# LongTarget/Fasim-LongTarget

Measured on AMD Instinct MI355X. Metric: SW Gcells/s (logical, whole job: stage 1+2+3 of the triplex scan), higher is better.
Workload: dtype u8

## Files before the change

### fasim-longtarget_amd/csrc/align.hip

```cpp
#include <hip/hip_runtime.h>
#include <stdint.h>
#include <stdlib.h>
#include "kernels.h"

namespace fasim {

typedef short v2s __attribute__((ext_vector_type(2)));
typedef unsigned short v2u __attribute__((ext_vector_type(2)));
typedef int v4i __attribute__((ext_vector_type(4)));

__device__ __forceinline__ v2s a_s(v2u x) { return __builtin_bit_cast(v2s, x); }
__device__ __forceinline__ v2u a_u(v2s x) { return __builtin_bit_cast(v2u, x); }
__device__ __forceinline__ int a_i(v2s x) { return __builtin_bit_cast(int, x); }
__device__ __forceinline__ int a_i(v2u x) { return __builtin_bit_cast(int, x); }
__device__ __forceinline__ v2u u_from(int x) { return __builtin_bit_cast(v2u, x); }
__device__ __forceinline__ v2s s_fromi(int x) { return __builtin_bit_cast(v2s, x); }

__device__ __forceinline__ v2u apk_subs(v2u a, v2u b) { v2u r; asm("v_pk_sub_u16 %0, %1, %2 clamp" : "=v"(r) : "v"(a), "v"(b)); return r; }
__device__ __forceinline__ v2u apk_subs_k(v2u a, uint32_t k) { v2u r; asm("v_pk_sub_u16 %0, %1, %2 clamp" : "=v"(r) : "v"(a), "s"(k)); return r; }
__device__ __forceinline__ v2u apk_ksubs(uint32_t k, v2u a) { v2u r; asm("v_pk_sub_u16 %0, %1, %2 clamp" : "=v"(r) : "s"(k), "v"(a)); return r; }
__device__ __forceinline__ v2u apk_minu(v2u a, v2u b) { v2u r; asm("v_pk_min_u16 %0, %1, %2" : "=v"(r) : "v"(a), "v"(b)); return r; }
__device__ __forceinline__ v2u apk_minu_k(v2u a, uint32_t k) { v2u r; asm("v_pk_min_u16 %0, %1, %2" : "=v"(r) : "v"(a), "s"(k)); return r; }
__device__ __forceinline__ v2u apk_maxu(v2u a, v2u b) { v2u r; asm("v_pk_max_u16 %0, %1, %2" : "=v"(r) : "v"(a), "v"(b)); return r; }

// ... 706 lines not shown
		if (i + band < end) end = i + band;
		if (j < beg || j > end) { status = 3; break; }
		const uint32_t nib = dir[(int64_t)(width_d * i + (j - x)) * 64];
		int dv;
		const int dE = (nib & 1) ? 3 : 2, dF = (nib & 2) ? 5 : 4;
		if (state == 0) dv = dE; else if (state == 1) dv = dF; else { const int dh = (nib >> 2) & 3; dv = dh == 0 ? 1 : (dh == 1 ? dE : dF); }
		if (dv == 1) { --i; --j; state = 2; op = 0; }
		else if (dv == 2) { --i; state = 0; op = 1; }
		else if (dv == 3) { --i; state = 2; op = 1; }
		else if (dv == 4) { --j; state = 1; op = 2; }
		else { --j; state = 2; op = 2; }
		if (op == prev_op) ++e;
		else {
			if (l >= ALIGN_MAX_CIGAR) { status = 4; break; }
			rc[l++] = cig(e, prev_op);
			prev_op = op; e = 1;
		}
	}
	if (status == 0) {
		if (op == 0) { if (l >= ALIGN_MAX_CIGAR) status = 4; else rc[l++] = cig(e + 1, 0); }
		else { if (l + 2 > ALIGN_MAX_CIGAR) status = 4; else { rc[l++] = cig(e, op); rc[l++] = cig(1, 0); } }
	}
	if (status == 0) {
		const uint32_t off = atomicAdd(pool_count, (uint32_t)l);
		if ((uint64_t)off + (uint64_t)l > (uint64_t)pool_cap) status = 4;
		else { o->cigar_off = off; for (int k = 0; k < l; k++) cigar_pool[off + k] = rc[l - 1 - k]; }
	}
	o->status = status;
	if (status != 0) return;
	o->sw_score = score;
	o->cigar_len = l;
}

hipError_t launch_finish(const uint8_t* tcodes, const uint8_t* qcodes, const FwdProb* probs, const FwdOut* fwd, const int32_t* order,
	int32_t nprob, uint8_t* dirs, AlignOutDev* out, uint32_t* cigar_pool, uint32_t pool_cap, uint32_t* pool_count, hipStream_t st)
{
	if (nprob <= 0) return hipSuccess;
	hipError_t err = hipMemsetAsync(pool_count, 0, sizeof(uint32_t), st);
	if (err != hipSuccess) return err;
	hipLaunchKernelGGL((k_finish_lds<64, 2048>), dim3((nprob + 63) / 64), dim3(64), 0, st, tcodes, qcodes, probs, fwd, order, nprob, dirs, out,
		cigar_pool, pool_cap, pool_count);
	return hipGetLastError();
}

hipError_t launch_finish_mid(const uint8_t* tcodes, const uint8_t* qcodes, const FwdProb* probs, const FwdOut* fwd, const int32_t* idx_list,
	int32_t nlist, uint8_t* dirs, AlignOutDev* out, uint32_t* cigar_pool, uint32_t pool_cap, uint32_t* pool_count, hipStream_t st)
{
	if (nlist <= 0) return hipSuccess;
	static bool attr_set = false;
	if (!attr_set) { (void)hipFuncSetAttribute((const void*)k_finish_lds<256, 16384>, hipFuncAttributeMaxDynamicSharedMemorySize, 64 * 1024); attr_set = true; }
	hipLaunchKernelGGL((k_finish_lds<256, 16384>), dim3((nlist + 63) / 64), dim3(64), 0, st, tcodes, qcodes, probs, fwd, idx_list, nlist, dirs, out,
		cigar_pool, pool_cap, pool_count);
	return hipGetLastError();
}

hipError_t launch_finish_big(const uint8_t* tcodes, const uint8_t* qcodes, const FwdProb* probs, const FwdOut* fwd,
	const int32_t* idx_list, int32_t nlist, uint8_t* scratch, int32_t scratch_cap, AlignOutDev* out, uint32_t* cigar_pool,
	uint32_t pool_cap, uint32_t* pool_count, hipStream_t st)
{
	if (nlist <= 0) return hipSuccess;
	hipLaunchKernelGGL(k_finish, dim3((nlist + 63) / 64), dim3(64), 0, st, tcodes, qcodes, probs, fwd, nlist, scratch, scratch_cap, out,
		cigar_pool, pool_cap, pool_count, idx_list);
	return hipGetLastError();
}

}
```

### fasim-longtarget_amd/csrc/engine.cpp

```cpp
#include "engine.h"

extern "C" {

void fasim_params_default(fasim_params* p)
{
	p->rule = 0; p->cutLength = 5000; p->strand = 0; p->overlapLength = 100; p->ntMin = 20; p->ntMax = 100000;
	p->scoreMin = 0.0f; p->minIdentity = 60.0f; p->minStability = 1.0f; p->penaltyT = -1000; p->penaltyC = 0;
	p->cDistance = 15; p->cLength = 50; p->classicSim = 0;
}

const char* fasim_last_error(const fasim_engine* e) { return e ? e->err.c_str() : g_last_error.c_str(); }

int fasim_engine_create(int device, fasim_engine** out) { return fasim_engine_create_ex(device, 0, out); }

int fasim_engine_create_ex(int device, int32_t flags, fasim_engine** out)
{
	if (!out) return fail(nullptr, FASIM_E_ARG, "null out pointer");
	*out = nullptr;
	const bool tune = !(flags & FASIM_CREATE_NO_PROCESS_TUNING);
	if (tune) setenv("GPU_MAX_HW_QUEUES", "8", 0);
	if (tune) {
		static const bool once = [] {
			const char* e = getenv("FASIM_MALLOPT");
			if (e && atoi(e) == 0) return false;
			(void)mallopt(M_MMAP_THRESHOLD, 32 * 1024 * 1024);
			(void)mallopt(M_TRIM_THRESHOLD, 0x7fffffff);
			(void)mallopt(M_TOP_PAD, 256 * 1024 * 1024);
			return true;
		}();
		(void)once;
	}
	int count = 0;
	hipError_t he = hipGetDeviceCount(&count);
	if (he != hipSuccess || count <= 0) return fail(nullptr, FASIM_E_NODEVICE, "no HIP device available (%s); this library has no CPU fallback", hipGetErrorString(he));
	if (device < 0 || device >= count) return fail(nullptr, FASIM_E_NODEVICE, "device %d out of range (%d devices)", device, count);
	{
		const char* e = getenv("FASIM_BLOCKING_SYNC");
		if (tune && !(e && atoi(e) == 0)) { (void)hipSetDevice(device); (void)hipSetDeviceFlags(hipDeviceScheduleBlockingSync); (void)hipGetLastError(); }
	}
	fasim_engine* E = new fasim_engine();
	E->device = device;
	he = hipSetDevice(device);
	if (he == hipSuccess) he = hipStreamCreate(&E->st);
	if (he != hipSuccess) { int rc = fail(nullptr, FASIM_E_NODEVICE, "cannot initialise device %d: %s", device, hipGetErrorString(he)); delete E; return rc; }
	E->lut1 = make_lut(true); E->lut2 = make_lut(false);
	std::vector<uint8_t> lut(48 * 256);
	build_enc_lut(lut.data());
	if (upload(E, E->enc_lut, lut.data(), lut.size()) || E->counter.ensure(64) != hipSuccess) { delete E; return FASIM_E_HIP; }
	unsigned hc = std::thread::hardware_concurrency();
	const char* env = getenv("FASIM_HOST_THREADS");
	E->host_threads = env ? std::max(1, atoi(env)) : (int)std::min(96u, std::max(1u, hc * 3 / 8));
	E->host_threads_total = E->host_threads;
	E->host_threads_explicit = env != nullptr;
	const char* v1 = getenv("FASIM_SCAN_V1");
	E->scan_v1 = v1 && atoi(v1) != 0;
	const char* a1 = getenv("FASIM_ALIGN_V1");
	E->align_v1 = a1 && atoi(a1) != 0;
	const char* sw = getenv("FASIM_STRIPED_WINDOW");
	E->striped_window = sw && atoi(sw) != 0;
	*out = E;
	return FASIM_OK;
}

void fasim_engine_destroy(fasim_engine* e)
{
	if (!e) return;
	for (fasim_engine* w : e->workers) fasim_engine_destroy(w);
	e->workers.clear();
	(void)hipSetDevice(e->device);
	DevBuf* bufs[] = { &e->q1, &e->q2, &e->enc_lut, &e->counter, &e->dna, &e->seg_start, &e->seg_len, &e->enc_ids, &e->tcodes,
		&e->colmax, &e->probs, &e->max_out, &e->unit_len, &e->stage1, &e->hits, &e->hits_total, &e->hit_off, &e->hit_cnt, &e->thr,
		&e->ends, &e->bprobs, &e->bout, &e->scratch, &e->dna_res, &e->colmax16, &e->unit_ids, &e->flags, &e->stage1_in, &e->hits2,
		&e->fprobs, &e->ftasks, &e->fstream, &e->fout, &e->aout, &e->cigpool, &e->cigcount, &e->forder, &e->scratch2, &e->boundary, &e->fboundary, &e->unit_hz,
		&e->unit_first, &e->hz_cols, &e->hz_plan, &e->hz_base, &e->hz_items, &e->snap, &e->hz_state, &e->hz_rows, &e->hz_chunk, &e->hz_src, &e->hz_zero,
		&e->qsim, &e->sim_min, &e->sim_row, &e->sim_ev, &e->sim_cnt, &e->sim_nodes,
		&e->ublk, &e->btarget, &e->bidx, &e->bcounts, &e->blist[0], &e->blist[1], &e->blist[2], &e->bslots[0], &e->bslots[1], &e->bslots[2],
		&e->bprev, &e->lane_ub, &e->fzones, &e->fubslot, &e->bdec, &e->btab, &e->swin };
	for (auto& t : e->timed) { (void)hipEventDestroy(t.a); (void)hipEventDestroy(t.b); }
	for (hipEvent_t ev : e->ev_pool) (void)hipEventDestroy(ev);
	for (DevBuf* b : bufs) b->release();
	if (e->pin_dna) (void)hipHostFree(e->pin_dna);
	if (e->pin_sim) (void)hipHostFree(e->pin_sim);
	if (e->st) (void)hipStreamDestroy(e->st);
	delete e;
}

int fasim_set_option(fasim_engine* E, const char* key, int32_t value)
{
	if (!E || !key) return fail(E, FASIM_E_ARG, "null argument");
	if (!strcmp(key, "workers")) E->opt_workers = value > 0 ? value : 0;
	else if (!strcmp(key, "seg_batch")) E->opt_seg_batch = value > 0 ? value : 0;
	else if (!strcmp(key, "taper")) E->opt_taper = value;
	else if (!strcmp(key, "heavy_gate")) E->opt_gate = value;
	else if (!strcmp(key, "hazard_chunks")) E->hz_chunks = value;
	else if (!strcmp(key, "hazard_snapshots")) E->hz_snap = value;
	else if (!strcmp(key, "hazard_chunk_cols")) E->hz_target = value > 0 ? std::max(64, value) : 0;
	else if (!strcmp(key, "hazard_hot_weight")) E->hz_hot_w = value > 0 ? std::min(32, value) : 0;
	else if (!strcmp(key, "host_threads")) { if (value > 0) { E->host_threads = value; E->host_threads_total = value; E->host_threads_explicit = true; } }
	else if (!strcmp(key, "numa_affinity")) E->opt_numa = value != 0;
	else if (!strcmp(key, "band")) E->opt_band = value;
	else if (!strcmp(key, "striped_window")) E->striped_window = value > 0;
	else return fail(E, FASIM_E_ARG, "unknown option %s", key);
	return FASIM_OK;
}

static int refuse_long_query(fasim_engine* E, int64_t len, int index)
{
	char which[32] = "";
	if (index >= 0) snprintf(which, sizeof which, " (query %d)", index);
	return fail(E, FASIM_E_UNSUPPORTED, "query of %lld nt%s exceeds the limit of %d nt: above it the reference's 16-bit stage-1 pass "
		"overruns its fixed workspace (stats.h:397) and its output is undefined", (long long)len, which, FASIM_MAX_QUERY);
}

int fasim_set_query(fasim_engine* E, const char* rna, int32_t len)
{
	if (!E) return fail(nullptr, FASIM_E_ARG, "null engine");
	if (!rna || len <= 0) return fail(E, FASIM_E_ARG, "empty query");
	if (len > FASIM_MAX_QUERY) return refuse_long_query(E, len, -1);
	HIPOK(hipSetDevice(E->device));
	E->rna.assign(rna, rna + len);
	E->m = len;
	std::vector<uint8_t> c1(len), c2(len);
	E->query_acgt = true;
	for (int i = 0; i < len; i++) {
		c1[i] = code1(rna[i]); c2[i] = code2(rna[i]);
		const char c = rna[i];
		if (!(c == 'A' || c == 'C' || c == 'G' || c == 'T' || c == 'a' || c == 'c' || c == 'g' || c == 't')) E->query_acgt = false;
	}
	std::vector<uint8_t> cs(len);
	for (int i = 0; i < len; i++) cs[i] = sim_code(rna[i]);
	int rc = upload(E, E->q1, c1.data(), len);
	if (!rc) rc = upload(E, E->q2, c2.data(), len);
	if (!rc) rc = upload(E, E->qsim, cs.data(), len);
// ... 399 lines not shown
```

### fasim-longtarget_amd/csrc/engine.h

```cpp
#pragma once
#include <hip/hip_runtime.h>

#include <algorithm>
#include <atomic>
#include <chrono>
#include <sched.h>
#include <malloc.h>
#include <cstdarg>
#include <cstdio>
#include <cstdlib>
#include <cstring>
#include <deque>
#include <memory>
#include <string>
#include <condition_variable>
#include <mutex>
#include <thread>
#include <vector>

#include "../../include/fasim_hip.h"
#include "device_types.h"
#include "host_post.h"
#include "kernels.h"

// ... 22 lines not shown

inline double now_s() { return std::chrono::duration<double>(std::chrono::steady_clock::now().time_since_epoch()).count(); }

struct HostProf {
	static constexpr int N = 32;
	double t[N] = { 0 }; const char* name[N] = { nullptr };
	bool on = false;
	std::mutex mu;
	void add(int i, const char* nm, double dt) { if (on) { std::lock_guard<std::mutex> g(mu); t[i] += dt; name[i] = nm; } }
	void dump() { if (!on) return; for (int i = 0; i < N; i++) if (name[i]) fprintf(stderr, "[fasim prof] %-60s %12.6f\n", name[i], t[i]); }
	void reset() { for (int i = 0; i < N; i++) { t[i] = 0; name[i] = nullptr; } }
};
inline HostProf g_prof;
static inline double thread_cpu_s() { timespec ts; clock_gettime(CLOCK_THREAD_CPUTIME_ID, &ts); return (double)ts.tv_sec + 1e-9 * (double)ts.tv_nsec; }
struct CpuScope { int i; const char* nm; double t0; CpuScope(int i_, const char* n) : i(i_), nm(n), t0(g_prof.on ? thread_cpu_s() : 0.0) {} ~CpuScope() { if (g_prof.on) g_prof.add(i, nm, thread_cpu_s() - t0); } };
struct ProfScope { int i; const char* nm; double t0; ProfScope(int i_, const char* n) : i(i_), nm(n), t0(now_s()) {} ~ProfScope() { g_prof.add(i, nm, now_s() - t0); } };


struct fasim_engine {
	int device = 0;
	hipStream_t st = nullptr;
	std::string err;
	std::string rna;
	int m = 0;
	int snap_units = 0, snap_per_unit = 0;
	ScoreLut lut1, lut2;
	DevBuf q1, q2, enc_lut, counter, dna, seg_start, seg_len, enc_ids, tcodes, colmax, probs, max_out, unit_len,
		stage1, hits, hits_total, hit_off, hit_cnt, thr, ends, bprobs, bout, scratch, colmax16, unit_ids, flags, stage1_in, hits2,
		fprobs, ftasks, fstream, fout, aout, cigpool, cigcount, forder, scratch2, boundary, fboundary, unit_hz,
		unit_first, hz_cols, hz_plan, hz_base, hz_items, snap, hz_state, hz_rows, hz_chunk, hz_src, hz_zero,
		qsim, sim_min, sim_row, sim_ev, sim_cnt, sim_nodes,
		sim_req, sim_pairs, sim_used, sim_rounds, sim_col, sim_rowst, sim_state, sim_usedc, sim_debug, sim_nodes_in, sim_nodes_out, sim_out;
	bool align_v1 = false;
	std::vector<fasim_engine*> workers;
	struct HeavyGate { std::mutex m; std::condition_variable cv; int in_flight = 0; int cap = 3; };
	HeavyGate own_gate;
	HeavyGate* gate = nullptr;
	int host_threads_total = 1;
	int host_threads_share_total = 1;
	bool host_threads_explicit = false;
	int scan_workers = 1;
	std::atomic<int>* sim_in_flight = nullptr;
	std::atomic<int>* active_workers = nullptr;
	int sim_threads = 1;
	int opt_workers = 0, opt_seg_batch = 0;
	int opt_taper = -1, opt_gate = -1;
	int hz_chunks = -1, hz_snap = -1, hz_target = 0, hz_hot_w = 0;
	bool query_acgt = true;
	bool scan_v1 = false;
	int host_threads = 1;
	std::string dna_host;
	DevBuf dna_res;
	void* pin_dna = nullptr; size_t pin_cap = 0;
	void* pin_sim = nullptr; size_t pin_sim_cap = 0;
	struct Timed { hipEvent_t a, b; int family; };
	std::vector<Timed> timed;
	std::vector<hipEvent_t> ev_pool;
	double kernel_ms[FASIM_KERNEL_FAMILIES] = { 0 };
	int64_t kernel_launches[FASIM_KERNEL_FAMILIES] = { 0 };
	DevBuf ublk, btarget, bidx, bcounts, blist[3], bslots[3], bprev, lane_ub, fzones, fubslot, bdec, btab;
	int ublk_units = 0, ublk_blocks = 0;
	int opt_band = -1;
	int opt_numa = 1;
	DevBuf swin;
	bool striped_window = false;
	int64_t sw_probs = 0;
// ... 226 lines not shown
```

### fasim-longtarget_amd/csrc/engine_scan.cpp

```cpp
#include "engine.h"
#include <memory>

int sim_forward_units(fasim_engine* E, const uint8_t* tcodes_dev, int tstride, const int32_t* unit_len_dev, const int32_t* unit_len_host,
	int first, int nrun, const int64_t* min_scores, std::atomic<int>* ready, std::vector<std::vector<fasim_sim_node>>& lists)
{
	static_assert(sizeof(SimNodeDev) == sizeof(fasim_sim_node) && SIM_K == FASIM_SIM_K, "node layout");
	if (nrun <= 0) return FASIM_OK;
	int maxlen = 1;
	for (int u = 0; u < nrun; u++) maxlen = std::max(maxlen, unit_len_host[first + u]);
	if (E->m > 65534 || maxlen > 65534) return fail(E, FASIM_E_UNSUPPORTED, "the SIM forward sweep holds start points in 16 bits: query %d / target %d nt is too long", E->m, maxlen);
	const int64_t row_stride = (maxlen + 2 + 15) & ~15;
	const uint32_t cap = (uint32_t)((maxlen + 15) & ~15);
	ProfScope fwd_wall(13, "-F forward sweep (k_sim_forward slices), wall");
	DevBuf& d_min = E->sim_min; DevBuf& d_row = E->sim_row; DevBuf& d_ev = E->sim_ev; DevBuf& d_cnt = E->sim_cnt; DevBuf& d_nodes = E->sim_nodes;
	int rc = upload(E, d_min, min_scores, sizeof(int64_t) * nrun); if (rc) return rc;
	int per_slice = 1024;
	{
		size_t free_b = 0, total_b = 0;
		const size_t unit_b = (size_t)64 * cap * sizeof(SimEvent) + (size_t)2 * row_stride * sizeof(uint64_t);
		if (hipMemGetInfo(&free_b, &total_b) == hipSuccess) {
			const size_t have = std::min<size_t>(((size_t)96 << 30) / (size_t)std::max(1, E->scan_workers), E->sim_ev.cap + free_b / 3);
			per_slice = (int)std::max<size_t>(256, std::min<size_t>(8192, have / unit_b));
		}
		const int nslices = (nrun + per_slice - 1) / per_slice;
// ... 496 lines not shown
			}
			if (tiles > 16) seg_batch = std::max<int64_t>(1, seg_batch * 16 / tiles);
		}
		std::vector<std::pair<int64_t, int64_t>> chunks;
		{
			int64_t b0 = seg_first; const int64_t b_end = seg_first + seg_count;
			const int64_t taper_from = b_end - seg_count * taper_pct / 100;
			while (b0 < b_end) {
				int64_t len = (taper_pct > 0 && b0 >= taper_from) ? std::max<int64_t>(1, seg_batch / 2) : seg_batch;
				len = std::min(len, b_end - b0);
				chunks.push_back({ b0, b0 + len });
				b0 += len;
			}
		}
		struct Item { int q; int64_t b0, b1; };
		std::vector<Item> items;
		items.reserve(chunks.size() * (size_t)nquery);
		for (int q = 0; q < nquery; q++) for (const auto& c : chunks) items.push_back({ q, c.first, c.second });
		nworkers = (int)std::min<size_t>((size_t)nworkers, items.size());
		while ((int)E->workers.size() < nworkers - 1) {
			fasim_engine* w = nullptr;
			int rc = fasim_engine_create(E->device, &w); if (rc) return fail(E, rc, "cannot create worker engine: %s", fasim_last_error(nullptr));
			E->workers.push_back(w);
		}
		std::atomic<int> active_workers(nworkers), sim_active(0);
		std::vector<fasim_engine*> ws(1, E);
		for (int k = 0; k < nworkers - 1; k++) ws.push_back(E->workers[k]);
		{
			const char* envg = getenv("FASIM_HEAVY_GATE");
			E->own_gate.cap = E->opt_gate >= 0 ? E->opt_gate : (envg ? atoi(envg) : 4);
		}
		for (fasim_engine* w : ws) {
			w->gate = (ws.size() > 1 && E->own_gate.cap > 0) ? &E->own_gate : nullptr;
			w->scan_v1 = E->scan_v1; w->align_v1 = E->align_v1; w->striped_window = E->striped_window;
			w->hz_chunks = E->hz_chunks; w->hz_snap = E->hz_snap; w->hz_target = E->hz_target; w->hz_hot_w = E->hz_hot_w; w->opt_band = E->opt_band;
			w->host_threads = std::max(1, E->host_threads_total / nworkers);
			w->host_threads_share_total = E->host_threads_total; w->active_workers = &active_workers; w->sim_in_flight = &sim_active; w->scan_workers = (int)ws.size();
			{
				const int all = E->host_threads_explicit ? E->host_threads_total : usable_cores();
				w->sim_threads = std::max(1, all / (int)std::max<size_t>(1, std::min<size_t>((size_t)nworkers, items.size()) / 4));
			}
			HIPOK(hipSetDevice(E->device));
			int rc = upload(w, w->enc_ids, encs.data(), sizeof(int) * nenc); if (rc) return rc;
			drain_timed(w);
			for (int k = 0; k < FASIM_KERNEL_FAMILIES; k++) { w->kernel_ms[k] = 0; w->kernel_launches[k] = 0; }
			w->sw_probs = 0; w->sw_ms = 0.0;
		}
		std::vector<std::vector<HostTriplex>> per_item(items.size());
		std::vector<fasim_scan_stats> ist(items.size());
		for (auto& x : ist) memset(&x, 0, sizeof x);
		std::vector<double> it0(items.size(), 0.0), it1(items.size(), 0.0);
		std::vector<int> wrc(ws.size(), FASIM_OK);
		std::atomic<size_t> next(0);
		auto run = [&](size_t wi) {
			CpuScope cpu(28, "CPU seconds: worker threads themselves (HIP calls, lists, decisions)");
			(void)hipSetDevice(E->device);
			fasim_engine* w = ws[wi];
			for (;;) {
				const size_t c = next.fetch_add(1);
				if (c >= items.size()) { active_workers.fetch_sub(1); break; }
				const Item& itx = items[c];
				const std::string& rq = queries[(size_t)itx.q];
				it0[c] = now_s();
				BatchCtx ctx;
				int r = FASIM_OK;
				if (w->rna != rq) {
					r = fasim_set_query(w, rq.data(), (int)rq.size());
// ... 69 lines not shown
```

### fasim-longtarget_amd/csrc/engine_stage3.cpp

```cpp
#include "engine.h"


int run_finish(fasim_engine* E, const UnitBatch& B, const std::vector<WindowProb>& W, const std::vector<FwdOut>& fo,
	std::vector<AlignResult>& out, std::vector<uint32_t>& cigars, std::vector<char>& status);
bool align_v2_fits(const fasim_engine* E, const std::vector<WindowProb>& W);
int run_fwd(fasim_engine* E, const UnitBatch& B, const std::vector<WindowProb>& W, std::vector<FwdOut>& fo, bool word, const FwdZones* Z = nullptr);

int run_align(fasim_engine* E, const UnitBatch& B, const std::vector<WindowProb>& W, std::vector<AlignResult>& out,
	std::vector<uint32_t>& cigars, fasim_scan_stats* stats)
{
	const int n = (int)W.size();
	out.assign(n, AlignResult());
	if (!n) return FASIM_OK;
	ProfScope ps(6, "run_align (exact) total");
	std::vector<StripedProb> probs(n);
	for (int k = 0; k < n; k++) {
		probs[k].tbase = (int64_t)W[k].unit * B.tstride; probs[k].t0 = W[k].t0; probs[k].ref_len = W[k].len;
		probs[k].q_len = E->m; probs[k].unit = k; probs[k].aux = 0; probs[k].pad = 0;
	}
	HIPOK(E->ends.ensure(sizeof(AlignEnds) * n));
	int rc = run_striped(E, MODE_ALIGN, false, probs, false, tcv(E), E->m);
	if (rc) return rc;
	std::vector<AlignEnds> ends(n);
	HIPOK(hipMemcpyAsync(ends.data(), E->ends.p, sizeof(AlignEnds) * n, hipMemcpyDeviceToHost, E->st));
// ... 349 lines not shown
		const AlignEnds& e = ends[i];
		if (e.ref_begin < 0 || e.read_begin < 0 || e.score_rev >= 255) { f.flags |= 1; continue; }
		f.score = e.score_rev < f.score ? e.score_rev : f.score;
		f.ref_begin = e.ref_begin; f.read_begin = e.read_begin; f.flags |= 2;
	}
	return FASIM_OK;
}

int run_finish(fasim_engine* E, const UnitBatch& B, const std::vector<WindowProb>& W, const std::vector<FwdOut>& fo,
	std::vector<AlignResult>& out, std::vector<uint32_t>& cigars, std::vector<char>& status)
{
	const int n = (int)W.size();
	out.assign(n, AlignResult()); status.assign(n, 0);
	if (!n) return FASIM_OK;
	ProfScope ps(4, "run_finish total");
	std::vector<FwdProb> probs(n);
	for (int k = 0; k < n; k++) { probs[k].tbase = (int64_t)W[k].unit * B.tstride + W[k].t0; probs[k].len = W[k].len; probs[k].stream_off = 0; }
	const int scratch_cap = 16384;
	int rc = upload_async(E, E->fprobs, probs.data(), sizeof(FwdProb) * n); if (rc) return rc;
	rc = upload_async(E, E->fout, fo.data(), sizeof(FwdOut) * n); if (rc) return rc;
	HIPOK(E->aout.ensure(sizeof(AlignOutDev) * n));
	const size_t pool_cap = (size_t)n * 12 + 4096;
	HIPOK(E->cigpool.ensure(pool_cap * sizeof(uint32_t)));
	HIPOK(E->cigcount.ensure(64));
	hipError_t he;
	std::vector<int32_t> order(n);
	{
		std::vector<int32_t> cnt(1026, 0);
		for (int k = 0; k < n; k++) cnt[std::min(1024, std::max(0, fo[k].score)) + 1]++;
		for (int b = 1; b < 1026; b++) cnt[b] += cnt[b - 1];
		for (int k = 0; k < n; k++) order[cnt[std::min(1024, std::max(0, fo[k].score))]++] = k;
		rc = upload_async(E, E->forder, order.data(), sizeof(int32_t) * n); if (rc) return rc;
	}
	HIPOK(E->scratch.ensure((size_t)((n + 63) / 64) * 64 * 2048));
	{ TimedScope ts(E, 3);
	he = launch_finish(tcv(E), E->q2.as<uint8_t>(), E->fprobs.as<FwdProb>(), E->fout.as<FwdOut>(),
		E->forder.as<int32_t>(), n, E->scratch.as<uint8_t>(), E->aout.as<AlignOutDev>(), E->cigpool.as<uint32_t>(), (uint32_t)pool_cap,
		E->cigcount.as<uint32_t>(), E->st); }
	if (he != hipSuccess) return fail(E, FASIM_E_HIP, "finish launch failed: %s", hipGetErrorString(he));
	std::vector<AlignOutDev> ao(n);
	uint32_t pool_used = 0;
	HIPOK(hipMemcpyAsync(ao.data(), E->aout.p, sizeof(AlignOutDev) * n, hipMemcpyDeviceToHost, E->st));
	HIPOK(hipMemcpyAsync(&pool_used, E->cigcount.p, sizeof pool_used, hipMemcpyDeviceToHost, E->st));
	HIPOK(hipStreamSynchronize(E->st));
	{
		std::vector<int32_t> mid;
		for (int k = 0; k < n; k++) if (ao[k].status == 2) mid.push_back(k);
		if (!mid.empty()) {
			if (g_prof.on) g_prof.add(30, "finish: alignments sent to the 64 KB LDS pass (count)", 1e-6 * mid.size());
			rc = upload(E, E->unit_ids, mid.data(), sizeof(int32_t) * mid.size()); if (rc) return rc;
			HIPOK(E->scratch2.ensure((size_t)((mid.size() + 63) / 64) * 64 * 16384));
			{ TimedScope ts(E, 3);
			he = launch_finish_mid(tcv(E), E->q2.as<uint8_t>(), E->fprobs.as<FwdProb>(), E->fout.as<FwdOut>(), E->unit_ids.as<int32_t>(), (int)mid.size(),
				E->scratch2.as<uint8_t>(), E->aout.as<AlignOutDev>(), E->cigpool.as<uint32_t>(), (uint32_t)pool_cap, E->cigcount.as<uint32_t>(), E->st); }
			if (he != hipSuccess) return fail(E, FASIM_E_HIP, "finish (64 KB LDS) launch failed: %s", hipGetErrorString(he));
			HIPOK(hipMemcpyAsync(ao.data(), E->aout.p, sizeof(AlignOutDev) * n, hipMemcpyDeviceToHost, E->st));
			HIPOK(hipMemcpyAsync(&pool_used, E->cigcount.p, sizeof pool_used, hipMemcpyDeviceToHost, E->st));
			HIPOK(hipStreamSynchronize(E->st));
		}
	}
	{
		const int caps[2] = { scratch_cap, 1 << 20 };
		for (int pass = 0; pass < 2; pass++) {
			std::vector<int32_t> big;
			for (int k = 0; k < n; k++) if (ao[k].status == 2) big.push_back(k);
			if (big.empty()) break;
			if (g_prof.on) g_prof.add(17 + pass, pass ? "finish: alignments sent to the 1 MB pass (count)" : "finish: alignments sent to the 16 KB pass (count)", 1e-6 * big.size());
			rc = upload(E, E->unit_ids, big.data(), sizeof(int32_t) * big.size()); if (rc) return rc;
			const size_t per_launch = std::max<size_t>(64, ((size_t)2 << 30) / (size_t)caps[pass]);
			HIPOK(E->scratch2.ensure(std::min(big.size(), per_launch) * (size_t)caps[pass]));
			for (size_t b0 = 0; b0 < big.size(); b0 += per_launch) {
				const size_t cnt = std::min(per_launch, big.size() - b0);
				{ TimedScope ts(E, 6);
				he = launch_finish_big(tcv(E), E->q2.as<uint8_t>(), E->fprobs.as<FwdProb>(), E->fout.as<FwdOut>(),
					E->unit_ids.as<int32_t>() + b0, (int)cnt, E->scratch2.as<uint8_t>(), caps[pass], E->aout.as<AlignOutDev>(),
					E->cigpool.as<uint32_t>(), (uint32_t)pool_cap, E->cigcount.as<uint32_t>(), E->st); }
				if (he != hipSuccess) break;
			}
			if (he != hipSuccess) return fail(E, FASIM_E_HIP, "finish (global scratch) launch failed: %s", hipGetErrorString(he));
			HIPOK(hipMemcpyAsync(ao.data(), E->aout.p, sizeof(AlignOutDev) * n, hipMemcpyDeviceToHost, E->st));
			HIPOK(hipMemcpyAsync(&pool_used, E->cigcount.p, sizeof pool_used, hipMemcpyDeviceToHost, E->st));
			HIPOK(hipStreamSynchronize(E->st));
		}
	}
	if (pool_used > pool_cap) pool_used = (uint32_t)pool_cap;
	const uint32_t pool_base = (uint32_t)cigars.size();
	cigars.resize((size_t)pool_base + pool_used);
// ... 283 lines not shown
```

### fasim-longtarget_amd/csrc/kernels.h

```cpp
#pragma once
#include <hip/hip_runtime.h>
#include <vector>
#include "device_types.h"

namespace fasim {

enum StripedMode { MODE_PRE = 0, MODE_MAX1 = 1, MODE_ALIGN = 2, MODE_REV = 3 };

constexpr int HAZARD_MAX_CHUNKS = 512;
struct StripedLaunch {
	const uint8_t* tcodes;
	const uint8_t* qcodes;
	const StripedProb* probs;
	int32_t nprob;
	uint32_t* counter;
	ScoreLut lut;
	int32_t max_qlen;
	uint8_t* colmax;
	uint16_t* colmax_w = nullptr;
	int32_t* max_out;
	AlignEnds* ends;
	const uint16_t* state = nullptr; int32_t state_rows = 0; const int32_t* chunk_cols = nullptr; const int32_t* chunk_base = nullptr; uint8_t* chunk_rows = nullptr; int32_t row_stride = 0;
	int32_t* chunk_out = nullptr;
	bool spread = false;
// ... 31 lines not shown
	int32_t* unit_first = nullptr;
	uint32_t* snap = nullptr;
	int32_t snap_per_unit = 0;
	const ScanDumpItem* dump_items = nullptr;
	const int32_t* dump_cols = nullptr;
	uint16_t* dump_state = nullptr;
	uint16_t* ublk = nullptr;
	int32_t ublk_blocks = 0;
};
constexpr int SCAN_UBLK_STEPS = 64;
inline int scan_ublk_blocks(int tstride) { return (tstride + 127 + SCAN_UBLK_STEPS - 1) / SCAN_UBLK_STEPS; }
constexpr int SYSTOLIC_MAX_TILES = 31;
int systolic_vs(int m);
int systolic_tiles(int m);
bool systolic_fits(int m);
int systolic_snap_dwords(int m);
hipError_t launch_scan(const ScanLaunch& L, hipStream_t st);
hipError_t launch_scan_post(const uint16_t* colmax16, const int32_t* unit_ids, int32_t nwork, const int32_t* unit_len,
	int32_t tstride, const int32_t* stage1_in, uint32_t* hits, uint32_t hits_cap, uint32_t* hits_total, int32_t* hit_off,
	int32_t* hit_cnt, int32_t* thr_out, int32_t* stage1_out, int32_t* flags, const int32_t* unit_hz, hipStream_t st);
hipError_t launch_max16(const uint16_t* colmax16, const int32_t* unit_ids, int32_t nwork, const int32_t* unit_len,
	int32_t tstride, int32_t* out, hipStream_t st);

struct FwdLaunch {
	const uint8_t* stream; const FwdProb* probs; const int32_t* task_first; int32_t ntask; uint32_t* counter;
	const uint8_t* qcodes; int32_t m; FwdOut* out;
	uint4* boundary;
	int32_t word;
	uint16_t* lane_ub = nullptr; const int32_t* ub_slot = nullptr;
};
hipError_t launch_build_stream(const uint8_t* tcodes, const FwdProb* probs, int32_t nprob, uint8_t* stream, const uint32_t* zones, hipStream_t st);
hipError_t launch_align_fwd(const FwdLaunch& L, hipStream_t st);
hipError_t launch_finish(const uint8_t* tcodes, const uint8_t* qcodes, const FwdProb* probs, const FwdOut* fwd, const int32_t* order,
	int32_t nprob, uint8_t* dirs, AlignOutDev* out, uint32_t* cigar_pool, uint32_t pool_cap, uint32_t* pool_count, hipStream_t st);

hipError_t launch_finish_mid(const uint8_t* tcodes, const uint8_t* qcodes, const FwdProb* probs, const FwdOut* fwd, const int32_t* idx_list,
	int32_t nlist, uint8_t* dirs, AlignOutDev* out, uint32_t* cigar_pool, uint32_t pool_cap, uint32_t* pool_count, hipStream_t st);
hipError_t launch_finish_big(const uint8_t* tcodes, const uint8_t* qcodes, const FwdProb* probs, const FwdOut* fwd,
	const int32_t* idx_list, int32_t nlist, uint8_t* scratch, int32_t scratch_cap, AlignOutDev* out, uint32_t* cigar_pool,
	uint32_t pool_cap, uint32_t* pool_count, hipStream_t st);

struct BandTry { int32_t prob, r0, theta_min, nq; };
constexpr int BAND_SLOT_COLS = 208;
constexpr int BAND_MAX_ZONES = 32;
constexpr int BAND_COUNT_COLS = 3 * BAND_MAX_ZONES, BAND_COUNT_HOT = BAND_COUNT_COLS + 3, BAND_COUNT_NOBAND = BAND_COUNT_COLS + 4, BAND_COUNTS = 128;
struct BandSelLaunch {
	const FwdProb* probs; const int32_t* target; const int32_t* idx; int32_t n, tstride;
	const uint16_t* ublk; int32_t ublk_blocks; int32_t m; const uint8_t* tcodes;
	const uint16_t* prev_ub = nullptr; const int32_t* prev = nullptr;
	BandTry* list[3]; uint16_t* slots[3]; uint32_t list_cap;
	int4* dec;
	uint32_t* counts;
	uint32_t* cursors;
	FwdOut* out; int32_t class_mask;
	int32_t debug = 0;
};
struct BandZoneTab { int32_t zbase, first, count, wg, nwg; };
struct BandLaunch { const BandTry* list; const uint16_t* slots; const BandZoneTab* tab; int32_t nwg, cls; const uint8_t* qcodes; int32_t m; FwdOut* out; };
int band_profile_lanes(int m);
int band_zone_stride(int m);
int band_classes(int m);
std::vector<BandZoneTab> band_plan(int m, int cls, const uint32_t* zone_count, const uint32_t* zone_first);
hipError_t launch_band_decide(const BandSelLaunch& L, hipStream_t st);
hipError_t launch_band_emit(const BandSelLaunch& L, hipStream_t st);
hipError_t launch_align_band(const BandLaunch& L, hipStream_t st);

hipError_t launch_sim_forward(const SimFwdArgs& a, int32_t nunit, hipStream_t st);
hipError_t launch_sim_resweep(const SimResweepArgs& a, int32_t nunit, bool few_units, hipStream_t st);

}
// ... 1 lines not shown
```

Before: 3035.

## Run finish traceback with 16-lane groups per alignment using DPP prefix scans

Adds a new finish kernel where each alignment is handled by a 16-lane group (four or three per wavefront) instead of one thread per alignment. The reverse pass and the banded fill are vectorised across lanes, with DPP row shifts and prefix-max scans resolving the gap dependency. Direction bytes are kept in per-group LDS rather than global scratch. The old thread-per-alignment kernels remain behind a FASIM_FINISH_V1 switch. This adds cross-lane overhead and more complex control flow, and the finish stage may be only a small share of whole-job time.

```diff
diff --git a/fasim-longtarget_amd/csrc/align.hip b/fasim-longtarget_amd/csrc/align.hip
--- a/fasim-longtarget_amd/csrc/align.hip
+++ b/fasim-longtarget_amd/csrc/align.hip
@@ -762,23 +762,266 @@
 	o->cigar_len = l;
 }
 
+constexpr int FG_CACHE = 256;
+constexpr int FG_NEG = -1000000;
+
+template <int FG_RING, int FG_W, int FG_CELLS>
+struct FinishGroupLds {
+	uint8_t dir[FG_CELLS];
+	int32_t g[FG_RING];
+	int32_t e[FG_RING];
+	int32_t hp[FG_W];
+	int32_t ep[FG_W];
+	uint8_t qc[FG_CACHE];
+	uint8_t tc[FG_CACHE];
+};
+
+__device__ __forceinline__ void lds_order() { asm volatile("" ::: "memory"); }
+__device__ __forceinline__ int row_shr(int old, int x, int n)
+{
+	switch (n) {
+	case 1: return __builtin_amdgcn_update_dpp(old, x, 0x111, 0xf, 0xf, false);
+	case 2: return __builtin_amdgcn_update_dpp(old, x, 0x112, 0xf, 0xf, false);
+	case 4: return __builtin_amdgcn_update_dpp(old, x, 0x114, 0xf, 0xf, false);
+	default: return __builtin_amdgcn_update_dpp(old, x, 0x118, 0xf, 0xf, false);
+	}
+}
+__device__ __forceinline__ int row_prefix_max(int x)
+{
+	x = max(x, row_shr(FG_NEG, x, 1));
+	x = max(x, row_shr(FG_NEG, x, 2));
+	x = max(x, row_shr(FG_NEG, x, 4));
+	return max(x, row_shr(FG_NEG, x, 8));
+}
+__device__ __forceinline__ uint32_t group_ballot(bool p) { return (uint32_t)(__ballot(p) >> (threadIdx.x & 48)) & 0xffffu; }
+__device__ __forceinline__ int group_lane15(int x) { return __shfl(x, (int)(threadIdx.x & 48) | 15, 64); }
+
+template <int FG_RING, class Lds>
+__device__ int reverse_pass_g16(const uint8_t* __restrict__ tw, const uint8_t* __restrict__ q, int S, int ref_end, int read_end,
+	Lds& L, int lane, int* ref_begin, int* read_begin)
+{
+	const int R = read_end + 1, C = ref_end + 1;
+	const int g0 = swsc(L.qc[0], L.tc[0]);
+	if (g0 <= 0) return 1;
+	if (g0 == S) { *ref_begin = ref_end; *read_begin = read_end; return 0; }
+	int lo = 0, hi = 0;
+	if (lane == 0) { L.g[0] = g0; L.e[0] = FG_NEG; }
+	for (int j = 1; j < C; j++) {
+		if (hi - lo + 2 >= FG_RING) return 2;
+		const int tcode = j < FG_CACHE ? L.tc[j] : tw[ref_end - j];
+		const int colrest = C - 1 - j;
+		int Fc = FG_NEG, Dc = FG_NEG;
+		int nlo = -1, nhi = -1;
+		for (int c0 = lo; c0 < R; c0 += 16) {
+			const int i = c0 + lane;
+			const bool valid = i < R, in = i <= hi;
+			lds_order();
+			const int gp = in ? L.g[i & (FG_RING - 1)] : FG_NEG;
+			const int ep = in ? L.e[i & (FG_RING - 1)] : FG_NEG;
+			const int qcode = !valid ? 4 : (i < FG_CACHE ? L.qc[i] : q[read_end - i]);
+			const int diag = row_shr(Dc, gp, 1);
+			const int e = max(ep - GAP_EXT, gp - GAP_OPEN);
+			const int h0 = max(diag + swsc(qcode, tcode), e);
+			const int rest = min(R - 1 - i, colrest);
+			const int a = (h0 > 0 && h0 + 5 * rest >= S) ? h0 - GAP_OPEN : FG_NEG;
+			const int ex = row_shr(FG_NEG, row_prefix_max(a + GAP_EXT * lane), 1);
+			int F = max(Fc - GAP_EXT * lane, ex - GAP_EXT * (lane - 1));
+			if (F <= 0) F = FG_NEG;
+			int g = max(h0, F), ev = e;
+			if (g <= 0 || g + 5 * rest < S) g = FG_NEG;
+			if (ev <= 0 || ev + 5 * rest < S) ev = FG_NEG;
+			int Fn = max(F - GAP_EXT, a);
+			if (Fn <= 0) Fn = FG_NEG;
+			const uint32_t hit = group_ballot(valid && g == S);
+			const uint32_t brk = group_ballot(valid && i > hi && Fn <= 0 && gp <= 0);
+			const uint32_t ring = group_ballot(valid && i - lo + 2 >= FG_RING);
+			const uint32_t live = group_ballot(valid && (g > 0 || ev > 0));
+			const uint32_t any = hit | brk | ring;
+			const int s = any ? __builtin_ctz(any) : 15;
+			if ((hit >> s) & 1) { *ref_begin = ref_end - j; *read_begin = read_end - (c0 + s); return 0; }
+			lds_order();
+			if (valid && lane <= s) { L.g[i & (FG_RING - 1)] = g; L.e[i & (FG_RING - 1)] = ev; }
+			const uint32_t lv = live & (s >= 15 ? 0xffffu : ((2u << s) - 1));
+			if (lv) { if (nlo < 0) nlo = c0 + __builtin_ctz(lv); nhi = c0 + 31 - __builtin_clz(lv); }
+			if ((brk >> s) & 1) break;
+			if (any) return 2;
+			Fc = group_lane15(Fn); Dc = group_lane15(gp);
+		}
+		if (nlo < 0) return 1;
+		lo = nlo; hi = nhi;
+	}
+	return 1;
+}
+
+template <int FG_RING, int FG_W, int FG_CELLS, int GROUPS>
+__global__ void __launch_bounds__(64) k_finish_g16(const uint8_t* __restrict__ tcodes, const uint8_t* __restrict__ qcodes,
+	const FwdProb* __restrict__ probs, const FwdOut* __restrict__ fwd, const int32_t* __restrict__ order, int32_t nprob,
+	AlignOutDev* __restrict__ out, uint32_t* __restrict__ cigar_pool, uint32_t pool_cap, uint32_t* __restrict__ pool_count)
+{
+	__shared__ FinishGroupLds<FG_RING, FG_W, FG_CELLS> lds[GROUPS];
+	const int lane = threadIdx.x & 15, grp = threadIdx.x >> 4;
+	const int gid = blockIdx.x * GROUPS + grp;
+	if (grp >= GROUPS || gid >= nprob) return;
+	auto& L = lds[grp];
+	const int pi = order ? order[gid] : gid;
+	const FwdProb pb = probs[pi];
+	const FwdOut fo = fwd[pi];
+	AlignOutDev* o = out + pi;
+	const bool lead = lane == 0;
+	if (lead) {
+		o->sw_score = 0; o->ref_begin = 0; o->ref_end = fo.ref_end; o->query_begin = 0; o->query_end = fo.read_end; o->cigar_len = 0;
+		o->cigar_off = 0;
+	}
+	if (fo.flags & 1) { if (lead) o->status = 10; return; }
+	if (fo.score <= 0 || fo.ref_end < 0) { if (lead) o->status = 0; return; }
+	const uint8_t* tw = tcodes + pb.tbase;
+	{
+		const int nq = min(fo.read_end + 1, FG_CACHE), nt = min(fo.ref_end + 1, FG_CACHE);
+		uint8_t vq[FG_CACHE / 16], vt[FG_CACHE / 16];
+#pragma unroll
+		for (int r = 0; r < FG_CACHE / 16; r++) {
+			vq[r] = qcodes[fo.read_end - min(lane + 16 * r, nq - 1)];
+			vt[r] = tw[fo.ref_end - min(lane + 16 * r, nt - 1)];
+		}
+#pragma unroll
+		for (int r = 0; r < FG_CACHE / 16; r++) { L.qc[lane + 16 * r] = vq[r]; L.tc[lane + 16 * r] = vt[r]; }
+		lds_order();
+	}
+	int ref_begin = fo.ref_begin, read_begin = fo.read_begin;
+	if (!(fo.flags & 2)) {
+		if (fo.score >= 148 && fo.score < 255 - BIAS) { if (lead) o->status = 11; return; }
+		const int r = reverse_pass_g16<FG_RING>(tw, qcodes, fo.score, fo.ref_end, fo.read_end, L, lane, &ref_begin, &read_begin);
+		if (r) { if (lead) o->status = r == 2 ? 2 : 11; return; }
+	}
+	if (lead) { o->ref_begin = ref_begin; o->query_begin = read_begin; }
+	const int refLen = fo.ref_end - ref_begin + 1, readLen = fo.read_end - read_begin + 1, score = fo.score;
+	int band = (refLen > readLen ? refLen - readLen : readLen - refLen) + 1;
+	int maxv = 0, width_d = 0;
+	do {
+		const int width = band * 2 + 3;
+		width_d = band * 2 + 1;
+		if (width + 1 > FG_W || width_d * readLen > FG_CELLS) { if (lead) o->status = 2; return; }
+		int mx = 0;
+		for (int i = 0; i < readLen; i++) {
+			const int beg = max(0, i - band), end = min(refLen - 1, i + band);
+			const int pend = i == 0 ? -1 : (i <= band + 1 ? end - 1 : min(refLen - 1, i - 1 + band));
+			const int rk = readLen - 1 - i;
+			const int rd = rk < FG_CACHE ? L.qc[rk] : qcodes[fo.read_end - rk];
+			lds_order();
+			int hc = 0, fc = 0;
+			int dc = (i > 0 && beg >= 1) ? L.hp[(beg - 1) & (FG_W - 1)] : 0;
+			for (int j0 = beg; j0 <= end; j0 += 16) {
+				const int j = j0 + lane;
+				const bool valid = j <= end;
+				lds_order();
+				const bool upin = j <= pend;
+				const int hup = upin ? L.hp[j & (FG_W - 1)] : 0, eup = upin ? L.ep[j & (FG_W - 1)] : 0;
+				const int ck = refLen - 1 - j;
+				const int rc = !valid ? 4 : (ck < FG_CACHE ? L.tc[ck] : tw[fo.ref_end - ck]);
+				const int hdiag = row_shr(dc, hup, 1);
+				int t1 = hup - GAP_OPEN, t2 = eup - GAP_EXT;
+				const int ev = t1 > t2 ? t1 : t2;
+				const int de = t1 > t2 ? 1 : 0;
+				const int e1 = ev > 0 ? ev : 0;
+				const int td = hdiag + swsc(rc, rd);
+				const int f0 = max(hc - GAP_OPEN, fc - GAP_EXT);
+				const int ex = row_shr(FG_NEG, row_prefix_max(max(e1, td) - GAP_OPEN + GAP_EXT * (lane + 1)), 1);
+				const int f = max(f0, ex) - GAP_EXT * lane;
+				const int f1 = f > 0 ? f : 0;
+				t1 = e1 > f1 ? e1 : f1;
+				const int hv = t1 > td ? t1 : td;
+				const int dh = (t1 <= td) ? 0 : (e1 > f1 ? 1 : 2);
+				const int hl = row_shr(hc, hv, 1), fl = row_shr(fc, f, 1);
+				const int df = (hl - GAP_OPEN) > (fl - GAP_EXT) ? 1 : 0;
+				if (valid) {
+					if (hv > mx) mx = hv;
+					L.dir[width_d * i + (j - beg)] = (uint8_t)(de | (df << 1) | (dh << 2));
+				}
+				if (j0 + 16 <= end) { hc = group_lane15(hv); fc = group_lane15(f); dc = group_lane15(hup); }
+				lds_order();
+				if (valid) { L.hp[j & (FG_W - 1)] = hv; L.ep[j & (FG_W - 1)] = ev; }
+			}
+		}
+		for (int o2 = 8; o2 > 0; o2 >>= 1) mx = max(mx, __shfl_xor(mx, o2, 16));
+		maxv = max(maxv, mx);
+		band *= 2;
+		if (maxv < score && band > 4 * (refLen + readLen) + 16) { if (lead) o->status = 3; return; }
+	} while (maxv < score);
+	band /= 2;
+	if (!lead) return;
+	lds_order();
+	uint32_t* rc = reinterpret_cast<uint32_t*>(L.g);
+	int l = 0;
+	int i = readLen - 1, j = refLen - 1, e = 0, state = 2, op = 0, prev_op = 0, status = 0;
+	while (i > 0) {
+		const int x = i - band > 0 ? i - band : 0;
+		int beg = 0, end = refLen - 1;
+		if (i - band > beg) beg = i - band;
+		if (i + band < end) end = i + band;
+		if (j < beg || j > end) { status = 3; break; }
+		const uint32_t nib = L.dir[width_d * i + (j - x)];
+		int dv;
+		const int dE = (nib & 1) ? 3 : 2, dF = (nib & 2) ? 5 : 4;
+		if (state == 0) dv = dE; else if (state == 1) dv = dF; else { const int dh = (nib >> 2) & 3; dv = dh == 0 ? 1 : (dh == 1 ? dE : dF); }
+		if (dv == 1) { --i; --j; state = 2; op = 0; }
+		else if (dv == 2) { --i; state = 0; op = 1; }
+		else if (dv == 3) { --i; state = 2; op = 1; }
+		else if (dv == 4) { --j; state = 1; op = 2; }
+		else { --j; state = 2; op = 2; }
+		if (op == prev_op) ++e;
+		else {
+			if (l >= ALIGN_MAX_CIGAR) { status = 4; break; }
+			rc[l++] = cig(e, prev_op);
+			prev_op = op; e = 1;
+		}
+	}
+	if (status == 0) {
+		if (op == 0) { if (l >= ALIGN_MAX_CIGAR) status = 4; else rc[l++] = cig(e + 1, 0); }
+		else { if (l + 2 > ALIGN_MAX_CIGAR) status = 4; else { rc[l++] = cig(e, op); rc[l++] = cig(1, 0); } }
+	}
+	if (status == 0) {
+		const uint32_t off = atomicAdd(pool_count, (uint32_t)l);
+		if ((uint64_t)off + (uint64_t)l > (uint64_t)pool_cap) status = 4;
+		else { o->cigar_off = off; for (int k = 0; k < l; k++) cigar_pool[off + k] = rc[l - 1 - k]; }
+	}
+	o->status = status;
+	if (status != 0) return;
+	o->sw_score = score;
+	o->cigar_len = l;
+}
+
 hipError_t launch_finish(const uint8_t* tcodes, const uint8_t* qcodes, const FwdProb* probs, const FwdOut* fwd, const int32_t* order,
-	int32_t nprob, uint8_t* dirs, AlignOutDev* out, uint32_t* cigar_pool, uint32_t pool_cap, uint32_t* pool_count, hipStream_t st)
+	int32_t nprob, uint8_t* dirs, AlignOutDev* out, uint32_t* cigar_pool, uint32_t pool_cap, uint32_t* pool_count, bool v1, hipStream_t st)
 {
 	if (nprob <= 0) return hipSuccess;
 	hipError_t err = hipMemsetAsync(pool_count, 0, sizeof(uint32_t), st);
 	if (err != hipSuccess) return err;
+	if (!v1) {
+		hipLaunchKernelGGL((k_finish_g16<64, 32, 2048, 4>), dim3((nprob + 3) / 4), dim3(64), 0, st, tcodes, qcodes, probs, fwd, order, nprob, out, cigar_pool,
+			pool_cap, pool_count);
+		return hipGetLastError();
+	}
 	hipLaunchKernelGGL((k_finish_lds<64, 2048>), dim3((nprob + 63) / 64), dim3(64), 0, st, tcodes, qcodes, probs, fwd, order, nprob, dirs, out,
 		cigar_pool, pool_cap, pool_count);
 	return hipGetLastError();
 }
 
 hipError_t launch_finish_mid(const uint8_t* tcodes, const uint8_t* qcodes, const FwdProb* probs, const FwdOut* fwd, const int32_t* idx_list,
-	int32_t nlist, uint8_t* dirs, AlignOutDev* out, uint32_t* cigar_pool, uint32_t pool_cap, uint32_t* pool_count, hipStream_t st)
+	int32_t nlist, uint8_t* dirs, AlignOutDev* out, uint32_t* cigar_pool, uint32_t pool_cap, uint32_t* pool_count, bool v1, hipStream_t st)
 {
 	if (nlist <= 0) return hipSuccess;
-	static bool attr_set = false;
-	if (!attr_set) { (void)hipFuncSetAttribute((const void*)k_finish_lds<256, 16384>, hipFuncAttributeMaxDynamicSharedMemorySize, 64 * 1024); attr_set = true; }
+	if (!v1) {
+		hipLaunchKernelGGL((k_finish_g16<256, 128, 16384, 3>), dim3((nlist + 2) / 3), dim3(64), 0, st, tcodes, qcodes, probs, fwd, idx_list,
+			nlist, out, cigar_pool, pool_cap, pool_count);
+		return hipGetLastError();
+	}
+	static bool attr_set[64] = {};
+	int dev = 0;
+	if (hipGetDevice(&dev) != hipSuccess || dev < 0 || dev >= 64) dev = -1;
+	if (dev < 0 || !attr_set[dev]) {
+		(void)hipFuncSetAttribute((const void*)k_finish_lds<256, 16384>, hipFuncAttributeMaxDynamicSharedMemorySize, 64 * 1024);
+		if (dev >= 0) attr_set[dev] = true;
+	}
 	hipLaunchKernelGGL((k_finish_lds<256, 16384>), dim3((nlist + 63) / 64), dim3(64), 0, st, tcodes, qcodes, probs, fwd, idx_list, nlist, dirs, out,
 		cigar_pool, pool_cap, pool_count);
 	return hipGetLastError();
diff --git a/fasim-longtarget_amd/csrc/engine.cpp b/fasim-longtarget_amd/csrc/engine.cpp
--- a/fasim-longtarget_amd/csrc/engine.cpp
+++ b/fasim-longtarget_amd/csrc/engine.cpp
@@ -56,6 +56,8 @@
 	E->scan_v1 = v1 && atoi(v1) != 0;
 	const char* a1 = getenv("FASIM_ALIGN_V1");
 	E->align_v1 = a1 && atoi(a1) != 0;
+	const char* f1 = getenv("FASIM_FINISH_V1");
+	E->finish_v1 = f1 && atoi(f1) != 0;
 	const char* sw = getenv("FASIM_STRIPED_WINDOW");
 	E->striped_window = sw && atoi(sw) != 0;
 	*out = E;
@@ -99,6 +101,7 @@
 	else if (!strcmp(key, "host_threads")) { if (value > 0) { E->host_threads = value; E->host_threads_total = value; E->host_threads_explicit = true; } }
 	else if (!strcmp(key, "numa_affinity")) E->opt_numa = value != 0;
 	else if (!strcmp(key, "band")) E->opt_band = value;
+	else if (!strcmp(key, "finish_v1")) E->finish_v1 = value > 0;
 	else if (!strcmp(key, "striped_window")) E->striped_window = value > 0;
 	else return fail(E, FASIM_E_ARG, "unknown option %s", key);
 	return FASIM_OK;
diff --git a/fasim-longtarget_amd/csrc/engine.h b/fasim-longtarget_amd/csrc/engine.h
--- a/fasim-longtarget_amd/csrc/engine.h
+++ b/fasim-longtarget_amd/csrc/engine.h
@@ -78,6 +78,7 @@
 		qsim, sim_min, sim_row, sim_ev, sim_cnt, sim_nodes,
 		sim_req, sim_pairs, sim_used, sim_rounds, sim_col, sim_rowst, sim_state, sim_usedc, sim_debug, sim_nodes_in, sim_nodes_out, sim_out;
 	bool align_v1 = false;
+	bool finish_v1 = false;
 	std::vector<fasim_engine*> workers;
 	struct HeavyGate { std::mutex m; std::condition_variable cv; int in_flight = 0; int cap = 3; };
 	HeavyGate own_gate;
diff --git a/fasim-longtarget_amd/csrc/engine_scan.cpp b/fasim-longtarget_amd/csrc/engine_scan.cpp
--- a/fasim-longtarget_amd/csrc/engine_scan.cpp
+++ b/fasim-longtarget_amd/csrc/engine_scan.cpp
@@ -552,7 +552,7 @@
 		}
 		for (fasim_engine* w : ws) {
 			w->gate = (ws.size() > 1 && E->own_gate.cap > 0) ? &E->own_gate : nullptr;
-			w->scan_v1 = E->scan_v1; w->align_v1 = E->align_v1; w->striped_window = E->striped_window;
+			w->scan_v1 = E->scan_v1; w->align_v1 = E->align_v1; w->finish_v1 = E->finish_v1; w->striped_window = E->striped_window;
 			w->hz_chunks = E->hz_chunks; w->hz_snap = E->hz_snap; w->hz_target = E->hz_target; w->hz_hot_w = E->hz_hot_w; w->opt_band = E->opt_band;
 			w->host_threads = std::max(1, E->host_threads_total / nworkers);
 			w->host_threads_share_total = E->host_threads_total; w->active_workers = &active_workers; w->sim_in_flight = &sim_active; w->scan_workers = (int)ws.size();
diff --git a/fasim-longtarget_amd/csrc/engine_stage3.cpp b/fasim-longtarget_amd/csrc/engine_stage3.cpp
--- a/fasim-longtarget_amd/csrc/engine_stage3.cpp
+++ b/fasim-longtarget_amd/csrc/engine_stage3.cpp
@@ -405,11 +405,11 @@
 		for (int k = 0; k < n; k++) order[cnt[std::min(1024, std::max(0, fo[k].score))]++] = k;
 		rc = upload_async(E, E->forder, order.data(), sizeof(int32_t) * n); if (rc) return rc;
 	}
-	HIPOK(E->scratch.ensure((size_t)((n + 63) / 64) * 64 * 2048));
+	if (E->finish_v1) HIPOK(E->scratch.ensure((size_t)((n + 63) / 64) * 64 * 2048));
 	{ TimedScope ts(E, 3);
 	he = launch_finish(tcv(E), E->q2.as<uint8_t>(), E->fprobs.as<FwdProb>(), E->fout.as<FwdOut>(),
 		E->forder.as<int32_t>(), n, E->scratch.as<uint8_t>(), E->aout.as<AlignOutDev>(), E->cigpool.as<uint32_t>(), (uint32_t)pool_cap,
-		E->cigcount.as<uint32_t>(), E->st); }
+		E->cigcount.as<uint32_t>(), E->finish_v1, E->st); }
 	if (he != hipSuccess) return fail(E, FASIM_E_HIP, "finish launch failed: %s", hipGetErrorString(he));
 	std::vector<AlignOutDev> ao(n);
 	uint32_t pool_used = 0;
@@ -422,10 +422,11 @@
 		if (!mid.empty()) {
 			if (g_prof.on) g_prof.add(30, "finish: alignments sent to the 64 KB LDS pass (count)", 1e-6 * mid.size());
 			rc = upload(E, E->unit_ids, mid.data(), sizeof(int32_t) * mid.size()); if (rc) return rc;
-			HIPOK(E->scratch2.ensure((size_t)((mid.size() + 63) / 64) * 64 * 16384));
+			if (E->finish_v1) HIPOK(E->scratch2.ensure((size_t)((mid.size() + 63) / 64) * 64 * 16384));
 			{ TimedScope ts(E, 3);
 			he = launch_finish_mid(tcv(E), E->q2.as<uint8_t>(), E->fprobs.as<FwdProb>(), E->fout.as<FwdOut>(), E->unit_ids.as<int32_t>(), (int)mid.size(),
-				E->scratch2.as<uint8_t>(), E->aout.as<AlignOutDev>(), E->cigpool.as<uint32_t>(), (uint32_t)pool_cap, E->cigcount.as<uint32_t>(), E->st); }
+				E->scratch2.as<uint8_t>(), E->aout.as<AlignOutDev>(), E->cigpool.as<uint32_t>(), (uint32_t)pool_cap, E->cigcount.as<uint32_t>(),
+				E->finish_v1, E->st); }
 			if (he != hipSuccess) return fail(E, FASIM_E_HIP, "finish (64 KB LDS) launch failed: %s", hipGetErrorString(he));
 			HIPOK(hipMemcpyAsync(ao.data(), E->aout.p, sizeof(AlignOutDev) * n, hipMemcpyDeviceToHost, E->st));
 			HIPOK(hipMemcpyAsync(&pool_used, E->cigcount.p, sizeof pool_used, hipMemcpyDeviceToHost, E->st));
diff --git a/fasim-longtarget_amd/csrc/kernels.h b/fasim-longtarget_amd/csrc/kernels.h
--- a/fasim-longtarget_amd/csrc/kernels.h
+++ b/fasim-longtarget_amd/csrc/kernels.h
@@ -87,10 +87,10 @@
 hipError_t launch_build_stream(const uint8_t* tcodes, const FwdProb* probs, int32_t nprob, uint8_t* stream, const uint32_t* zones, hipStream_t st);
 hipError_t launch_align_fwd(const FwdLaunch& L, hipStream_t st);
 hipError_t launch_finish(const uint8_t* tcodes, const uint8_t* qcodes, const FwdProb* probs, const FwdOut* fwd, const int32_t* order,
-	int32_t nprob, uint8_t* dirs, AlignOutDev* out, uint32_t* cigar_pool, uint32_t pool_cap, uint32_t* pool_count, hipStream_t st);
+	int32_t nprob, uint8_t* dirs, AlignOutDev* out, uint32_t* cigar_pool, uint32_t pool_cap, uint32_t* pool_count, bool v1, hipStream_t st);
 
 hipError_t launch_finish_mid(const uint8_t* tcodes, const uint8_t* qcodes, const FwdProb* probs, const FwdOut* fwd, const int32_t* idx_list,
-	int32_t nlist, uint8_t* dirs, AlignOutDev* out, uint32_t* cigar_pool, uint32_t pool_cap, uint32_t* pool_count, hipStream_t st);
+	int32_t nlist, uint8_t* dirs, AlignOutDev* out, uint32_t* cigar_pool, uint32_t pool_cap, uint32_t* pool_count, bool v1, hipStream_t st);
 hipError_t launch_finish_big(const uint8_t* tcodes, const uint8_t* qcodes, const FwdProb* probs, const FwdOut* fwd,
 	const int32_t* idx_list, int32_t nlist, uint8_t* scratch, int32_t scratch_cap, AlignOutDev* out, uint32_t* cigar_pool,
 	uint32_t pool_cap, uint32_t* pool_count, hipStream_t st);
```

Measured after the change: 3101, median of 6. 2.2% higher.
